# SouthPoleTelescope/CosmoMC

Hardware: AMD Instinct MI355X
Metric: fast-param likelihood evals/sec/node (plik_lite_TTTEEE ℓmax=2508); R-1 vs wall-clock (higher is better)
Workload: dtype f64; 1 GPU; plik_lite_TTTEEE + Planck2018 lensing fast-parameter Metropolis step (BASELINE configs[2] minus lowl): GetProposalFast + native plik_lite (613 bins, l<=2508, full binning + quadratic form) + CMBlikes lensing (9 bins, linear correction) + calPlanck prior + accept; walkers_per_gpu=1024, stream_groups=1, global_walkers=1024, nbins=613, lmax=2508, parallelism=walkers sharded over 1 rank(s), no per-step collective

## Files before the change

cosmomc_amd/_native.py:

```python
from __future__ import annotations

import ctypes as C
import os
import re
import subprocess

PKG = os.path.dirname(os.path.abspath(__file__))
ROOT = os.path.dirname(PKG)
LIB_PATH = os.environ.get("COSMOMC_AMD_LIB") or os.path.join(PKG, "lib", "libcosmomc_amd.so")
HEADER = os.path.join(ROOT, "include", "cosmomc_amd.h")

CMBL_LOGZERO = 1e30
N_FIELDS = 10

ERRORS = {0: "OK", -1: "bad argument", -2: "I/O error", -3: "format error", -4: "numerical error",
          -5: "HIP error", -6: "unsupported"}


class NativeError(RuntimeError):
    def __init__(self, code, msg):
        super().__init__(f"[{ERRORS.get(code, code)}] {msg}")
        self.code = code


# ... 75 lines not shown
        L.cmbl_clik_workspace_size.restype = sz
        L.cmbl_status.argtypes = [vp, C.POINTER(i), i]
        L.cmbs_walker_seed.argtypes = [i, i, i, C.POINTER(i), C.POINTER(i)]
        L.cmbs_create.argtypes = [C.POINTER(CmbsConfig), C.POINTER(vp), C.c_char_p, sz]
        L.cmbs_destroy.argtypes = [vp]
        L.cmbs_last_error.argtypes = [vp]
        L.cmbs_last_error.restype = C.c_char_p
        L.cmbs_set_covariance.argtypes = [vp, vp]
        L.cmbs_set_test_gaussian.argtypes = [vp, vp, vp]
        L.cmbs_add_likelihood.argtypes = [vp, vp, vp, vp, ll, ll]
        L.cmbs_set_start.argtypes = [vp, vp, vp]
        L.cmbs_step.argtypes = [vp, i, i, vp]
        L.cmbs_set_groups.argtypes = [vp, i]
        L.cmbs_set_binned_cache.argtypes = [vp, i]
        L.cmbs_history_host.argtypes = [vp, i, i, vp]
        L.cmbs_set_trial_theory.argtypes = [vp, i, vp, ll, ll]
        L.cmbs_step_drag.argtypes = [vp, i, d, THEORY_FN, vp, vp]
        L.cmbs_step_theory.argtypes = [vp, i, THEORY_FN, vp, vp]
        L.cmbs_refresh_theory.argtypes = [vp, THEORY_FN, vp, vp]
        L.cmbt_create.argtypes = [C.POINTER(CmbtConfig), C.POINTER(vp), C.c_char_p, sz]
        L.cmbt_destroy.argtypes = [vp]
        L.cmbt_last_error.argtypes = [vp]
        L.cmbt_last_error.restype = C.c_char_p
        L.cmbt_eval.argtypes = [vp, i, vp, ll, i, vp, ll, ll, vp, vp]
        L.cmbt_set_derived.argtypes = [vp, C.POINTER(CmbtDerivedConfig)]
        L.cmbt_derived_count.argtypes = [vp]
        L.cmbt_derived_eval.argtypes = [vp, i, vp, ll, i, vp, ll, vp, vp]
        L.cmbs_set_theory_calculator.argtypes = [vp, vp]
        L.cmbs_set_like_calculator.argtypes = [vp, i, vp]
        L.cmbg_create.argtypes = [vp, C.POINTER(CmbgConfig), C.POINTER(vp), C.c_char_p, sz]
        L.cmbg_destroy.argtypes = [vp]
        L.cmbg_last_error.argtypes = [vp]
        L.cmbg_last_error.restype = C.c_char_p
        L.cmbg_eval.argtypes = [vp, i, vp, ll, i, vp, vp, vp]
        L.cmbs_add_derived_likelihood.argtypes = [vp, vp]
        L.cmbs_collector_enable.argtypes = [vp, i]
        L.cmbs_collector_add.argtypes = [vp, vp, i, i, i, vp]
        L.cmbs_collector_state_host.argtypes = [vp, vp, vp, vp, vp]
        L.cmbs_collector_thin.argtypes = [vp, i, vp]
        L.cmbs_collector_moments.argtypes = [vp, vp, vp, vp]
        L.cmbs_collector_limits.argtypes = [vp, vp, i, d, vp, vp]
        L.cmbs_chain_moments.argtypes = [vp, i, i, vp, vp, vp]
        L.cmbs_enable_history.argtypes = [vp, i]
        L.cmbs_history_stats.argtypes = [vp, i, i, vp, vp, vp]
        L.cmbs_history_count.argtypes = [vp]
        L.cmbs_state.argtypes = [vp, C.POINTER(vp), C.POINTER(vp), C.POINTER(vp), C.POINTER(vp)]
        L.cmbs_get_state_host.argtypes = [vp, vp, vp, vp, vp]
        L.cmbs_state_bytes.argtypes = [vp]
        L.cmbs_state_bytes.restype = sz
        L.cmbs_save_state.argtypes = [vp, vp, sz]
        L.cmbs_load_state.argtypes = [vp, vp, sz]
        L.cmbs_history_restore.argtypes = [vp, i, i, vp, vp]
        L.cmbs_history_terms_host.argtypes = [vp, i, i, vp]
        L.cmbl_profile_enable.argtypes = [i]
        L.cmbl_profile_reset.argtypes = []
        L.cmbl_profile_read.argtypes = [C.c_char_p, C.POINTER(d), C.POINTER(ll)]
        _lib = L
    return _lib


def exported_symbols_from_header() -> list[str]:
    with open(HEADER) as f:
        txt = f.read()
    txt = re.sub(r"/\*.*?\*/", "", txt, flags=re.S)
    return sorted(set(re.findall(r"\b(cmb[ls]_[a-z_0-9]+)\s*\(", txt)))


def check(rc: int, handle=None, kind: str = "cmbl"):
    if rc != 0:
        msg = ""
        if handle is not None:
            fn = {"cmbl": lib().cmbl_last_error, "cmbs": lib().cmbs_last_error, "cmbt": lib().cmbt_last_error,
                  "cmbg": lib().cmbg_last_error}[kind]
            msg = (fn(handle) or b"").decode()
        raise NativeError(rc, msg)


def current_stream_ptr(device=None) -> int:
    import torch
    if device is None:
        try:
            return torch._C._cuda_getCurrentRawStream(torch._C._cuda_getDevice())
        except AttributeError:
            pass
    return torch.cuda.current_stream(device).cuda_stream


def require_gpu():
    import torch
    if not torch.cuda.is_available():
        raise RuntimeError("cosmomc_amd compute needs an MI355X (HIP) device; none visible")


def profile_enable(on: bool = True):
    lib().cmbl_profile_enable(int(on))


def profile_reset():
    lib().cmbl_profile_reset()


def profile_read(kernel: str):
    t, n = C.c_double(), C.c_longlong()
    lib().cmbl_profile_read(kernel.encode(), C.byref(t), C.byref(n))
    return t.value, n.value
```

cosmomc_amd/csrc/mhbody.h:

```cpp
#pragma once

template <bool ACCEPT, bool PROPOSE>
__device__ __forceinline__ void mh_body(const DevCfg &c, int fast_only, double *hist_row, double *hist_terms, int blk0,
                                        double *lds, int bx, const TailWait *tw = nullptr)
{
    if (c.lean.on) {
        mh_lean<ACCEPT, PROPOSE>(c, hist_row, hist_terms, blk0, lds, bx, tw);
        return;
    }
    const Rows &R = c.rows;
    const int lane = threadIdx.x % MB, grp = threadIdx.x / MB;
    const int wl64 = threadIdx.x & 63, wave = threadIdx.x >> 6, nwave = MH_THREADS / 64;
    const int wb = (blk0 + bx) * MB;
    const int w = wb + lane;
    const bool act = w < c.W;
    const size_t W = c.ld;
    const int nlk = (c.n_like + 1) & ~1;
    const int nd_st = c.stage_R ? R.ND : R.ND - R.RR;
    const int ni_st = c.stage_cyc ? R.NI : R.CYC;
    const int ntd = c.stage_cov ? c.tl.n_dbl : c.tl.covinv;
    double *sd = lds;
    double *lk = sd + (size_t)nd_st * MB;
    double *vc = lk + (size_t)nlk * MB;
    double *tq = vc + (size_t)c.max_blk * MB;
    double *dq = tq + (size_t)c.tq_rows * MB;
    double *td = dq + (size_t)c.def_cap * (QF_GROUPS + 1) * MB;
    int *si = reinterpret_cast<int *>(td + ((ntd + 31) & ~31));
    int *it = si + (size_t)ni_st * MB;
    int *ti = it + (size_t)(c.stage_cyc ? c.all_n : 0) * MB;
    int *oobw = ti + ((c.tl.n_int + 63) & ~63);
    double *zz = reinterpret_cast<double *>(oobw + MB);
    int *ndw = reinterpret_cast<int *>(zz + (size_t)c.np * MB);
    int *i0w = ndw + MB;
    if (threadIdx.x < MB) oobw[threadIdx.x] = 0;
    if (PROPOSE && c.rot_defer && bx == 0 && threadIdx.x == 0)
        c.rot_cnt[2 * (blk0 * MB / 64) + (c.rot_par ^ 1)] = 0;
    const bool skipR = !c.stage_R;
#define SROW(r) ((skipR && (r) >= R.R) ? (r) - R.RR : (r))

    STAMP(0);
    const int rEnd = R.R + R.RR;
    if (skipR) {
        dma_rows_f64(sd, 0, c.sd, 0, R.R, W, wb, wl64, wave, nwave);
        dma_rows_f64(sd, R.R, c.sd, rEnd, R.ND - rEnd, W, wb, wl64, wave, nwave);
    } else {
        dma_rows_f64(sd, 0, c.sd, 0, R.ND, W, wb, wl64, wave, nwave);
    }
    dma_rows_i32(si, c.si, ni_st, W, wb, wl64, wave, nwave);
    dma_words(td, c.tab_d, 2 * ntd, wl64, wave, nwave);
    dma_words(ti, c.tab_i, c.tl.n_int, wl64, wave, nwave);
    const bool pre_col = PROPOSE && fast_only && !c.stage_R && c.pre_blk >= 0;
    constexpr int NRQ = (MAXBLK + NV - 1) / NV;
    double rq[NRQ];
    int col = -1, ncol = 0;
    const bool rq_early = pre_col && c.pre_lp >= 0;
    if (rq_early && act) {
        ncol = c.pre_n;
        if (c.pre_lp % ncol != 0) col = c.pre_off + c.pre_lp;
#pragma unroll
        for (int u = 0; u < NRQ; u++) {
// ... 302 lines not shown
```

cosmomc_amd/csrc/mhlean.h:

```cpp
#pragma once

template <bool ACCEPT, bool PROPOSE>
__device__ __forceinline__ void mh_lean(const DevCfg &c, double *hist_row, double *hist_terms, int blk0, double *lds,
                                        int bx, const TailWait *tw)
{
    const Rows &R = c.rows;
    const LeanCfg &L = c.lean;
    const int lane = threadIdx.x % MB, grp = threadIdx.x / MB;
    const int wl64 = threadIdx.x & 63, wave = threadIdx.x >> 6, nwave = MH_THREADS / 64;
    const int wb = (blk0 + bx) * MB;
    const int w = wb + lane;
    const bool act = w < c.W;
    const size_t W = c.ld;
    const int np = c.np;
    const int nd_lo = R.R, nd_hi = R.ND - R.P;
    double *sd = lds;
    double *sp = sd + (size_t)nd_lo * MB;
    double *dq = sp + (size_t)nd_hi * MB;
    double *zz = dq + (size_t)MAXDEF * (QF_GROUPS + 1) * MB;
    int *si = reinterpret_cast<int *>(zz + (size_t)np * MB);
    int *oobw = si + 8 * MB;
    int *ndw = oobw + MB;
    int *i0w = ndw + MB;
    if (threadIdx.x < MB) oobw[threadIdx.x] = 0;
    if (PROPOSE && c.rot_defer && bx == 0 && threadIdx.x == 0)
        c.rot_cnt[2 * (blk0 * MB / 64) + (c.rot_par ^ 1)] = 0;

    STAMP(0);
    dma_rows_f64(sd, 0, c.sd, 0, nd_lo, W, wb, wl64, wave, nwave);
    dma_rows_f64(sd, nd_lo, c.sd, R.P, nd_hi, W, wb, wl64, wave, nwave);
    dma_rows_i32(si, c.si, 8, W, wb, wl64, wave, nwave);
    constexpr int PG = MAXP / NV;
    double lo[PG], hi[PG], mu[PG], sg[PG];
    const double *td = c.tab_d;
#pragma unroll
    for (int u = 0; u < PG; u++) {
        const int i = grp + u * NV;
        if (ACCEPT && i < np) {
            lo[u] = td[c.tl.pmin + i];
            hi[u] = td[c.tl.pmax + i];
            mu[u] = td[c.tl.pmean + i];
            sg[u] = td[c.tl.pstd + i];
        }
    }
    int pu[PG];
    if (ACCEPT && hist_row) {
#pragma unroll
        for (int u = 0; u < PG; u++) {
            const int i = grp + u * NV;
            if (i < c.n_used) pu[u] = c.tab_i[c.tl.params_used + i];
        }
    }
    if (tw) tail_wait(*tw, wb / 64);
    if (ACCEPT && c.n_def) {
        const int tile = wb / QF_TILE, col = wb % QF_TILE + lane;
        for (int d = 0; d < MAXDEF; d++) {
            if (d >= c.n_def) break;
            const double *tp = c.def_part[d] + (size_t)tile * c.def_items[d] * QF_TILE;
            double *row = dq + (size_t)d * (QF_GROUPS + 1) * MB;
            if (grp < QF_GROUPS) row[(size_t)grp * MB + lane] = qf_group_sum(tp, c.def_items[d], grp, col);
            if (grp == NV - 1) row[(size_t)QF_GROUPS * MB + lane] = (c.def_add[d] && act) ? c.def_add[d][w] : 0.0;
        }
    }
    double lk[MAXLIKE], ct[MAXLIKE];
    if (ACCEPT && grp == 0 && act) {
#pragma unroll
        for (int l = 0; l < MAXLIKE; l++)
            if (l < c.n_like) {
                lk[l] = c.like_terms[(size_t)l * W + w];
                if (hist_terms) ct[l] = c.cur_terms[(size_t)l * W + w];
            }
    }
    STAMP(1);
    asm volatile("s_waitcnt vmcnt(0)" ::: "memory");
    __syncthreads();
    const double *trial_l = sp + (size_t)np * MB + lane;
    if (ACCEPT && act) {
        int oob = 0;
#pragma unroll
        for (int u = 0; u < PG; u++) {
            const int i = grp + u * NV;
            if (i < np) {
                const double qv = trial_l[(size_t)i * MB];
                if (qv > hi[u] || qv < lo[u]) oob = 1;
                double z2 = 0.0;
                if (c.has_priors && sg[u] != 0.0) {
                    const double z = (qv - mu[u]) / sg[u];
                    z2 = z * z;
                }
                zz[(size_t)i * MB + lane] = z2;
            }
        }
        if (oob) atomicOr(&oobw[lane], 1);
    }
    if (ACCEPT) __syncthreads();
    STAMP(2);

    if (grp == 0 && act) {
        Rng r;
        r.u = Col<double>{sd + (size_t)R.U * MB + lane, MB};
        r.c = sd[(size_t)R.C * MB + lane];
        r.gset = sd[(size_t)R.G * MB + lane];
        r.i97 = si[(size_t)R.I97 * MB + lane];
        r.j97 = si[(size_t)R.J97 * MB + lane];
        r.iset = si[(size_t)R.ISET * MB + lane];
        r.nd = 0;
        const int i97_0 = r.i97;
        double *P = sp + lane;
        double *T = sp + (size_t)np * MB + lane;
        double cur = sp[(size_t)(2 * np) * MB + lane];
        double mult = sp[(size_t)(2 * np + 1) * MB + lane];
        int nacc = si[(size_t)R.NACC * MB + lane];
        bool moved = false;
        if (ACCEPT) {
            for (int d = 0; d < MAXDEF; d++) {
                if (d >= c.n_def) break;
                const double *row = dq + (size_t)d * (QF_GROUPS + 1) * MB;
                double v = qf_tree(row + lane, MB);
                if (c.def_add[d]) v = v + row[(size_t)QF_GROUPS * MB + lane];
                const int l = c.def_like[d];
#pragma unroll
                for (int q = 0; q < MAXLIKE; q++)
                    if (q == l) lk[q] = v;
                const_cast<double *>(c.like_terms)[(size_t)l * W + w] = v;
            }
            double like;
            if (oobw[lane]) like = LOGZERO;
            else {
                double main = 0.0;
                bool zero = false;
#pragma unroll
                for (int l = 0; l < MAXLIKE; l++)
                    if (l < c.n_like) {
                        if (lk[l] == LOGZERO) zero = true;
                        main += lk[l];
                    }
                if (zero) like = LOGZERO;
                else {
                    like = main / c.temperature;
                    if (c.has_priors) {
                        double pri = 0.0;
                        for (int i = 0; i < np; i++) pri += zz[(size_t)i * MB + lane];
                        like = like + (pri / 2.0) / c.temperature;
                    }
                }
            }
            bool acc = false;
            if (like != LOGZERO) {
                acc = cur > like;
                if (!acc) acc = (double)randexp1(r) > like - cur;
            }
            moved = acc;
            if (acc) {
                if (mult > 0) nacc += 1;
                mult = 1.0;
                for (int i = 0; i < np; i++) P[(size_t)i * MB] = T[(size_t)i * MB];
                cur = like;
#pragma unroll
                for (int l = 0; l < MAXLIKE; l++)
                    if (l < c.n_like) {
                        ct[l] = lk[l];
                        c.cur_terms[(size_t)l * W + w] = ct[l];
                    }
            } else {
                mult += 1.0;
            }
            c.si[(size_t)R.ACCF * W + w] = acc ? 1 : 0;
            c.si[(size_t)R.NACC * W + w] = nacc;
            c.sd[(size_t)R.L * W + w] = cur;
            c.sd[(size_t)R.M * W + w] = mult;
            if (hist_row) hist_row[(size_t)c.n_used * c.W + w] = cur;
            if (hist_terms) {
#pragma unroll
                for (int l = 0; l < MAXLIKE; l++)
                    if (l < c.n_like) hist_terms[(size_t)l * c.W + w] = ct[l];
            }
        }
        STAMP(3);
        if (PROPOSE) {
            if (!moved)
                for (int i = 0; i < np; i++) T[(size_t)i * MB] = P[(size_t)i * MB];
            (void)ranmar(r);
            const double r1 = (ranmar(r) - 0.5) >= 0.0 ? 1.0 : -1.0;
            double rf;
            if (ranmar(r) < 0.33) {
                rf = (double)randexp1(r);
            } else {
                rf = 0.0;
                const double g = gaussian1(r);
                rf += g * g;
                rf = sqrt(rf / 1);
            }
            const double scale = rf * c.propose_scale;
            const double v0 = r1 * scale;
#pragma unroll
            for (int j = 0; j < LEAN_MAXC; j++)
                if (j < L.nc) {
                    double s = 0.0;
                    s += L.map[j] * v0;
                    T[(size_t)L.chg[j] * MB] += s;
                }
            if (c.pub_on)
#pragma unroll
                for (int k = 0; k < 2; k++) {
                    const int pc = c.pub_pcal[k];
                    const double v = pc >= 0 ? T[(size_t)pc * MB] : 1.0;
                    __hip_atomic_store(c.calbuf + (size_t)k * W + w, v, __ATOMIC_RELAXED, __HIP_MEMORY_SCOPE_AGENT);
                    __hip_atomic_store(c.calbuf_next + (size_t)k * W + w,
                                       __longlong_as_double((long long)TP_PIPE_UNSET), __ATOMIC_RELAXED,
                                       __HIP_MEMORY_SCOPE_AGENT);
                }
            STAMP(4);
#pragma unroll
            for (int l = 0; l < MAXLIKE; l++)
#pragma unroll
                for (int q = 0; q < LEAN_MAXQ; q++)
                    if (l < c.n_like && q < L.nn[l])
                        c.like_nuis[l][(size_t)w * L.nn[l] + q] = T[(size_t)L.nuis[l][q] * MB];
            c.sd[(size_t)L.r_row * W + w] = r1;
            c.si[(size_t)(R.CYCLP + 2) * W + w] = 1;
            c.si[(size_t)L.cyc_row * W + w] = 1;
            c.si[(size_t)L.blklp_row * W + w] = 1;
            c.si[(size_t)R.PROT * W + w] = 0;
        }
        c.sd[(size_t)R.C * W + w] = r.c;
        c.sd[(size_t)R.G * W + w] = r.gset;
        c.si[(size_t)R.I97 * W + w] = r.i97;
        c.si[(size_t)R.J97 * W + w] = r.j97;
        c.si[(size_t)R.ISET * W + w] = r.iset;
        ndw[lane] = r.nd < 97 ? r.nd : 97;
        i0w[lane] = i97_0;
    }
    __syncthreads();
    STAMP(12);
    if (!act) return;
    {
        const int nd = ndw[lane], i0 = i0w[lane];
        for (int t = grp; t < nd; t += NV) {
            int p = i0 - 1 - t;
            if (p < 0) p += 97;
            c.sd[(size_t)(R.U + p) * W + w] = sd[(size_t)(R.U + p) * MB + lane];
        }
    }
    for (int i = grp; i < np; i += NV) {
        if (ACCEPT) c.sd[(size_t)(R.P + i) * W + w] = sp[(size_t)i * MB + lane];
        if (PROPOSE) c.sd[(size_t)(R.T + i) * W + w] = sp[(size_t)(np + i) * MB + lane];
    }
    if (ACCEPT && hist_row) {
#pragma unroll
        for (int u = 0; u < PG; u++) {
            const int i = grp + u * NV;
            if (i < c.n_used) hist_row[(size_t)i * c.W + w] = sp[(size_t)pu[u] * MB + lane];
        }
    }
    STAMP(5);
#ifdef CMAMD_STAMPS
    asm volatile("s_waitcnt vmcnt(0)" ::: "memory");
    STAMP(6);
#endif
}
```

cosmomc_amd/csrc/mhrng.h:

```cpp
#pragma once

template <class T> struct Col {
    T *p;
    int s;
    __device__ T &operator[](int i) const { return p[(size_t)i * s]; }
};


struct Rng {
    Col<double> u;
    double c;
    int i97, j97, iset;
    double gset;
    int nd = 0;
};

__device__ __forceinline__ double ranmar(Rng &r)
{
    double uni = r.u[r.i97 - 1] - r.u[r.j97 - 1];
    if (uni < 0.0) uni += 1.0;
    r.u[r.i97 - 1] = uni;
    if (--r.i97 == 0) r.i97 = 97;
    if (--r.j97 == 0) r.j97 = 97;
    r.nd++;
    const double cd = 7654321.0 / 16777216.0, cm = 16777213.0 / 16777216.0;
    r.c -= cd;
    if (r.c < 0.0) r.c += cm;
    uni -= r.c;
    if (uni < 0.0) uni += 1.0;
    return uni;
}

__device__ __forceinline__ double gaussian1(Rng &r)
{
    if (r.iset == 0) {
        double v1, v2, rr;
        do {
            v1 = 2.0 * ranmar(r) - 1.0;
            v2 = 2.0 * ranmar(r) - 1.0;
            rr = v1 * v1 + v2 * v2;
        } while (rr >= 1.0);
        const double fac = sqrt(-2.0 * log(rr) / rr);
        r.gset = v1 * fac;
        r.iset = 1;
        return v2 * fac;
    }
    r.iset = 0;
    return r.gset;
}

__device__ __forceinline__ float randexp1(Rng &r)
{
    const float alog2 = 0.6931471805599453f, a = 5.7133631526454228f, b = 3.4142135623730950f;
    const float c = -1.6734053240284925f, p = 0.9802581434685472f, aa = 5.6005707569738080f;
    const float bb = 3.3468106480569850f, hh = 0.0026106723602095f, dd = 0.0857864376269050f;
    float u = (float)ranmar(r);
    while (u <= 0.0f) u = (float)ranmar(r);
    float g = c;
    u = u + u;
    while (u < 1.0f) {
        g = g + alog2;
        u = u + u;
    }
    u = u - 1.0f;
    if (u <= p) return g + aa / (bb - u);
    for (;;) {
        u = (float)ranmar(r);
        const float y = a / (b - u);
        const float up = (float)ranmar(r);
        const float bu = b - u;
        if ((up * hh + dd) * (bu * bu) <= expf(-(y + c))) return g + y;
    }
}
```

cosmomc_amd/csrc/mhstep.h:

```cpp
#pragma once


static constexpr int UNI_WT = 4;

template <bool ACCEPT, bool PROPOSE>
__device__ __forceinline__ void mh_step_body(DevCfg &c, int fast_only, double *hist_row, double *hist_terms,
                                             StepTail &t, const int2 *__restrict__ rows, TailWait &tw, int nmh)
{
    extern __shared__ __attribute__((aligned(16))) double lds[];
    const int2 rr = rows[blockIdx.x >> 3];
    const int lb = rr.y * 8 + (blockIdx.x & 7);
    if (!ACCEPT && blockIdx.x == 0)
        for (int i = threadIdx.x; i < tw.ntiles; i += MH_THREADS) tw.cnt[i] = 0u;
#ifdef CMAMD_STAMPS
    const bool stamp = ACCEPT && threadIdx.x == 0 && blockIdx.x < 2048;
    const int slot = PROPOSE ? 0 : 1;
    if (stamp) {
        unsigned xcc;
        asm volatile("s_getreg_b32 %0, hwreg(HW_REG_XCC_ID)" : "=s"(xcc));
        g_uni_stamps[slot][blockIdx.x][0] = __builtin_amdgcn_s_memrealtime();
        g_uni_stamps[slot][blockIdx.x][2] = xcc & 15;
        g_uni_stamps[slot][blockIdx.x][4] = 0;
        g_uni_stamps[slot][blockIdx.x][5] = 0;
    }
    struct End {
        bool on;
        int role, slot;
        __device__ ~End() {
            if (on) {
                g_uni_stamps[slot][blockIdx.x][3] = __builtin_amdgcn_s_memrealtime();
                g_uni_stamps[slot][blockIdx.x][4] = role + 1;
            }
        }
    } end_{stamp, rr.x, slot};
#endif
    if (rr.x == TAIL_QF) {
        if (lb >= t.nq) return;
        int item_ix, tile;
        qf_place(lb, t.q.src.n_items, t.q.src.xcd_map, item_ix, tile);
        __builtin_amdgcn_s_setprio(2);
        qfs_body(lds, item_ix, tile, t.q);
        tail_arrive(tw, tile);
    } else if (rr.x == TAIL_GAUSS) {
        const int grows = (t.ng + 7) >> 3, q = (lb & 7) * grows + (lb >> 3);
        if (q >= t.ng) return;
        small_gauss_body<UNI_WT, true, true>(t.g, lds, q);
        tail_arrive(tw, q * UNI_WT / 64);
    } else if (rr.x == TAIL_PASS) {
        if (lb >= t.np) return;
        tp_vec_body<2, true, false>(t.tp, t.dl, t.ld_field, t.ld_walker, t.W, reinterpret_cast<char *>(lds), lb);
    } else if (lb < nmh) {
        __builtin_amdgcn_s_setprio(3);
        if (ACCEPT && t.fold_g) {
            small_gauss_body<MB, true, false>(t.g, lds, lb);
            asm volatile("s_waitcnt vmcnt(0)" ::: "memory");
            __syncthreads();
#ifdef CMAMD_STAMPS
            if (threadIdx.x == 0 && blockIdx.x < 2048)
                g_uni_stamps[PROPOSE ? 0 : 1][blockIdx.x][5] = __builtin_amdgcn_s_memrealtime();
#endif
        }
        mh_body<ACCEPT, PROPOSE>(c, fast_only, hist_row, hist_terms, 0, lds, lb, ACCEPT ? &tw : nullptr);
    }
}
```

cosmomc_amd/csrc/sampler.h:

```cpp
#pragma once

#include "common.h"
#include "steptail.h"
#include "theorypass.h"

namespace cmamd {

static constexpr int MAXLIKE = 8;
static constexpr int MAXGROUPS = 8;
static constexpr int MAXDEF = 2;

struct Rows {
    int U = 0;
    int C = 97;
    int G = 98;
    int R = 100;
    int RR;
    int P, T, L, M;
    int ND;
    int I97 = 0, J97 = 1, ISET = 2, FASTIX = 3, NACC = 4;
    int CYCLP = 5;
    int BLKLP = 8;
    int ACCF;
    int PROT;
// ... 26 lines not shown
    int has_priors, test_like, n_lin;
    int rot_defer;
    int *rot_list;
    int *rot_cnt;
    int rot_par;
    int rot_serial;
    Rows rows;
    TabLayout tl;
    const int *tab_i;
    const double *tab_d;
    double *sd;
    int *si;
    int stage_R;
    int pre_blk;
    int pre_lp;
    int pre_off, pre_n;
    int stage_cyc;
    int stage_cov;
    int *itmp_g;
    int tq_rows;
    int n_like;
    const double *like_terms;
    double *cur_terms;
    int like_nidx[MAXLIKE], like_nn[MAXLIKE];
    double *like_nuis[MAXLIKE];
    unsigned long long like_dep[MAXLIKE];
    int mask_on;
    int *like_flag;
    const double *like_out[MAXLIKE];
    int def_cap;
    int n_def;
    int def_like[MAXDEF], def_items[MAXDEF];
    const double *def_part[MAXDEF];
    const double *def_add[MAXDEF];
    int pub_on;
    int pub_pcal[2];
    double *calbuf;
    double *calbuf_next;
    int bin_on, bin_nused, bin_Np, bin_cal;
    const double *bin_S, *bin_X;
    double *bin_delta;
};

struct TailWait {
    unsigned int *cnt;
    unsigned int epoch;
    unsigned int epoch_g;
    int nq_items;
    int ng, gwt;
    int *status;
    int nosignal;
    int stamp_slot;
    int ntiles;
};

struct TheoryView {
    const double *dl = nullptr;
    long long ld_field = 0, ld_walker = 0;
    bool operator==(const TheoryView &o) const {
        return dl == o.dl && ld_field == o.ld_field && ld_walker == o.ld_walker;
    }
};

struct LikeSlot {
    cmbl_t *like;
    std::vector<int> nidx;
    TheoryView th;
};

}

struct cmbg;

struct cmbs {
    cmamd::DevCfg dc{};
    int W = 0, np = 0, n_used = 0;
    std::vector<int> params_used;
    std::string last_error;
    cmamd::DevBuf rot;
    std::vector<int> rot_par;
    std::vector<int> rot_lp;
    bool rot_fast_any = false;
    int rot_fast_n = 0;
    int stage_R_force = -1;
    cmamd::DevBuf tab_i, tab_d, sd, si, like_terms, cur_terms, ws, hist, hist_terms, mom, itmp_g;
    cmamd::DevBuf nuis_bufs[cmamd::MAXLIKE];
    std::vector<int> h_tab_i;
    std::vector<double> h_tab_d;
    std::vector<cmamd::LikeSlot> likes;
    std::vector<cmbg *> dlikes;
    bool drv_cur = false;
    int n_rows() const { return (int)(likes.size() + dlikes.size()); }
    std::vector<int> indices, proposer_for_index, blk_start, blk_n, blk_nchanged, used_params_changed_all;
    std::vector<int> blk_changed_off, blk_map_off, blk_R_off, changed;
    int all_n = 0, slow_n = 0, fast_n = 0, nblocks = 0, R_total = 0, map_total = 0;
    size_t mh_lds = 0;
    int hist_cap = 0, hist_count = 0;
    bool started = false;
    int n_groups = 1;
    std::vector<int> grp0{0};
    hipStream_t streams[cmamd::MAXGROUPS] = {};
    hipEvent_t events[cmamd::MAXGROUPS + 1] = {};
    cmamd::DevBuf ws_g[cmamd::MAXGROUPS];
    cmamd::DevBuf drag_dd, drag_di, like_terms2;
    cmamd::DevBuf like_ws2[cmamd::MAXLIKE];
    bool no_drag_pair = false;
    bool drag_hbm = false;
    cmamd::DevBuf nuis_bufs2[cmamd::MAXLIKE];
    cmamd::TheoryView end_theory[cmamd::MAXLIKE];
    long long num_drag = 0;
    cmbt *calc = nullptr;
    cmamd::DevBuf calc_fail;
    cmbt *like_calc[cmamd::MAXLIKE] = {};
    cmamd::DevBuf calc_fail2;
    bool theory_moved = false, theory_stale = false;
    struct Collector {
        cmamd::DevBuf samp, state, flag, wcount, steps;
        int cap = 0;
        bool enabled = false;
    } coll;
    cmamd::DevBuf like_flag, like_cnt;
    cmamd::DevBuf like_outc[cmamd::MAXLIKE], like_nuisc[cmamd::MAXLIKE], like_dlc[cmamd::MAXLIKE];
    std::vector<int> sparse_likes;
    bool mask_on = false;
    std::vector<int> defer_likes;
    cmamd::DevBuf like_ws[cmamd::MAXLIKE];
    int pending_def = 0;
    std::unique_ptr<cmamd::TheoryPass> tpass;
    int tp_like[2] = {-1, -1};
    cmamd::WinStage tp_stage[2];
    bool no_corun = false;
    cmamd::DevBuf pipe_cal;
    unsigned pipe_epoch = 0;
    int pipe_ready = 0;
    int pipe_mode = 3;
    cmamd::DevBuf tail_S[2][2];
    cmamd::DevBuf tail_rowcal;
    int tail_ready = 0;
    int tail_qf = -1, tail_g = -1;
    cmamd::DevBuf tail_cnt;
    size_t tail_cnt_bytes = 0;
    unsigned tail_epoch = 0;
    unsigned tail_epoch_g = 0;
    cmamd::StepTailPlan uni_plan[3];
    size_t uni_lds = 0;
    int tail_nosignal = 0;
    bool binned_cache = false;
    int *pipe_status_host = nullptr;
    int *pipe_status_dev = nullptr;
    hipEvent_t pipe_ev = nullptr;
    bool pipe_ev_pending = false;
    cmamd::DevBuf bin_S;
    size_t bin_lds = 0;
    int tp_why = 0;
    bool lean_off = false;
    ~cmbs() {
        if (pipe_status_host) (void)hipHostFree(pipe_status_host);
        if (pipe_ev) (void)hipEventDestroy(pipe_ev);
        for (auto &st : streams)
            if (st) (void)hipStreamDestroy(st);
        for (auto &e : events)
            if (e) (void)hipEventDestroy(e);
    }
};

namespace cmamd {
void sampler_set_groups(cmbs *s, int n_groups);
void sampler_check_pipe(cmbs *s, bool wait = false);
void rot_schedule_unknown(cmbs *s);
void sampler_chain_moments(cmbs *s, int first, int last, const double *gmean, double *out, hipStream_t stream);
void sampler_history_host(cmbs *s, int first, int count, double *out);
void sampler_set_trial_theory(cmbs *s, int like_index, double *dl_end, long long ld_field, long long ld_walker);
void sampler_step_drag(cmbs *s, int n_steps, double dragging_steps, cmbs_theory_fn fn, void *user, hipStream_t stream);
void sampler_step_theory(cmbs *s, int n_steps, cmbs_theory_fn fn, void *user, hipStream_t stream);
void sampler_refresh_theory(cmbs *s, cmbs_theory_fn fn, void *user, hipStream_t stream);
void sampler_set_theory_calculator(cmbs *s, cmbt *calc);
void sampler_set_like_calculator(cmbs *s, int like_index, cmbt *calc);
void sampler_add_derived_likelihood(cmbs *s, cmbg *g);
void sampler_collector_enable(cmbs *s, int samp_capacity);
void sampler_collector_add(cmbs *s, const int *steps, int nsteps, int min_update, int check_burn, hipStream_t st);
void sampler_collector_state_host(cmbs *s, int *start, int *count, int *burn, int *thin);
void sampler_collector_thin(cmbs *s, int limit, hipStream_t st);
void sampler_collector_moments(cmbs *s, const double *gmean, double *out, hipStream_t stream);
void sampler_collector_limits(cmbs *s, const int *params, int ncheck, double limfrac, double *out, hipStream_t stream);
size_t sampler_collector_bytes(const cmbs *s);
void sampler_collector_save(cmbs *s, void *buf);
void sampler_collector_load(cmbs *s, const void *buf);
}
```

cosmomc_amd/csrc/sampler.hip:

```cpp
#include <algorithm>
#include <cmath>
#include <cstring>

#include <cstdlib>

#include "plikbin.h"
#include "qfs_body.h"
#include "quadform.h"
#include "sampler.h"
#include "smallgauss.h"
#include "theorycalc.h"
#ifdef CMAMD_STAMPS
namespace cmamd {
__device__ unsigned long long g_uni_stamps[2][2048][6];
}
#endif
#include "theorypass_body.h"

namespace cmamd {

static constexpr double LOGZERO = CMBL_LOGZERO;
static constexpr int MAXP = 64;
static constexpr int MAXBLK = 32;
static constexpr int NB = 64;
// ... 58 lines not shown
        return;
    }
    const int w = b - nmh_pad;
    for (int i = pb.nused + (int)threadIdx.x; i < pb.Np; i += MH_THREADS)
        c.bin_delta[(size_t)w * pb.Np + i] = 0.0;
    double acc[3][2] = {};
#pragma unroll
    for (int f = 0; f < 3; f++) {
        if (f > 0) __syncthreads();
        if (!plik_bin_products(pb, lds, w, f)) continue;
        const double *P = lds - pb.fr.lo[f];
#pragma unroll
        for (int k = 0; k < 2; k++) {
            const int i = pb.fr.b0[f] + (int)threadIdx.x + k * MH_THREADS;
            if (i < pb.fr.b1[f]) {
                const BinInfo bi = pb.bins[i];
                for (int l = bi.lmin; l <= bi.lmax; l++) acc[f][k] += P[l];
            }
        }
    }
    if (threadIdx.x == 0) {
        double cl;
        for (long it = 0;; it++) {
            cl = __hip_atomic_load(c.calbuf + w, __ATOMIC_RELAXED, __HIP_MEMORY_SCOPE_AGENT);
            if ((unsigned long long)__double_as_longlong(cl) != TP_PIPE_UNSET) break;
            if (it == (1l << 20)) {
                pipe_giveup(status);
                break;
            }
            __builtin_amdgcn_s_sleep(24);
        }
        cal_s = cl;
    }
    __syncthreads();
    const double cl = cal_s, c2 = cl * cl;
    const bool rot = (unsigned long long)__double_as_longlong(cl) == TP_PIPE_ROT;
    double *out = (rot ? const_cast<double *>(c.bin_S) : c.bin_delta) + (size_t)w * pb.Np;
#pragma unroll
    for (int f = 0; f < 3; f++)
#pragma unroll
        for (int k = 0; k < 2; k++) {
            const int i = pb.fr.b0[f] + (int)threadIdx.x + k * MH_THREADS;
            if (pb.fr.hi[f] >= pb.fr.lo[f] && i < pb.fr.b1[f]) out[i] = rot ? acc[f][k] : pb.X[i] - acc[f][k] / c2;
        }
}

#include "mhstep.h"

template <bool ACCEPT, bool PROPOSE>
__global__ __launch_bounds__(MH_THREADS, 3) void mh_step_kernel(DevCfg c, int fast_only, double *hist_row,
                                                                double *hist_terms, StepTail t,
                                                                const int2 *__restrict__ rows, TailWait tw, int nmh)
{
    mh_step_body<ACCEPT, PROPOSE>(c, fast_only, hist_row, hist_terms, t, rows, tw, nmh);
}

template <bool ACCEPT, bool PROPOSE>
__global__ __launch_bounds__(MH_THREADS, 3) void mh_tail_kernel(DevCfg c, int fast_only, double *hist_row,
                                                                double *hist_terms, StepTail t,
                                                                const int2 *__restrict__ rows, TailWait tw, int nmh)
{
    mh_step_body<ACCEPT, PROPOSE>(c, fast_only, hist_row, hist_terms, t, rows, tw, nmh);
}

#include "mhrot.h"
#include "mhdrag.h"

__global__ void start_kernel(DevCfg c)
{
    const int w = blockIdx.x * blockDim.x + threadIdx.x;
    if (w >= c.W) return;
    const size_t W = c.ld;
    const Tabs t = make_tabs(c, c.tab_i, c.tab_d);
    Col<double> q{c.sd + (size_t)c.rows.T * W + w, c.ld};
    Col<const double> lk{c.like_terms + w, c.ld};
    c.sd[(size_t)c.rows.L * W + w] = target_like(c, t, q, lk);
    for (int l = 0; l < c.n_like; l++) c.cur_terms[(size_t)l * W + w] = lk[l];
    for (int i = 0; i < c.np; i++) c.sd[(size_t)(c.rows.P + i) * W + w] = q[i];
    c.sd[(size_t)c.rows.M * W + w] = 0.0;
    c.si[(size_t)c.rows.NACC * W + w] = 0;
}

__global__ void gather_nuis(const double *trial, int W, int ld, const int *nidx, int n_nuis, double *out)
{
    const int w = blockIdx.x * blockDim.x + threadIdx.x;
    if (w >= W) return;
    for (int k = 0; k < n_nuis; k++) out[(size_t)w * n_nuis + k] = trial[(size_t)nidx[k] * ld + w];
}

struct SparseSet {
    int like[MAXLIKE], nn[MAXLIKE];
    double *nuisc[MAXLIKE];
    int *map[MAXLIKE];
};

__global__ __launch_bounds__(1024) void like_compact_kernel(DevCfg c, SparseSet ss, int *__restrict__ cnt)
{
    __shared__ int wsum[16];
    const int b = blockIdx.x, l = ss.like[b], nn = ss.nn[b];
    int *flag = c.like_flag + (size_t)l * c.ld;
    const double *nuis = c.like_nuis[l];
    const int t = threadIdx.x, lane = t & 63, wave = t >> 6;
    const int chunk = (c.W + 1023) / 1024, w0 = t * chunk, w1 = min(c.W, w0 + chunk);
    int n = 0;
    for (int w = w0; w < w1; w++) n += flag[w] != 0;
    int v = n;
    for (int o = 1; o < 64; o <<= 1) {
        const int y = __shfl_up(v, o);
        if (lane >= o) v += y;
    }
    if (lane == 63) wsum[wave] = v;
    __syncthreads();
    int before = 0;
    for (int q = 0; q < wave; q++) before += wsum[q];
    int off = before + v - n;
// ... 866 lines not shown

static StepTail make_tail(cmbs *s, int rd, int wr) {
    StepTail t;
    const int W = s->W;
    t.W = W;
    if (rd >= 0) {
        const int qi = s->tp_like[s->tail_qf], gi = s->tp_like[s->tail_g];
        Like &Q = *s->likes[qi].like->like;
        Like &G = *s->likes[gi].like->like;
        if (!Q.qf_source(t.q.src, W, s->like_ws[qi].p)) fail(CMBL_ERR_ARG, "internal: step tail quadratic form");
        t.q.S = s->tail_S[rd][s->tail_qf].as<double>();
        t.q.nuis = s->dc.like_nuis[qi];
        t.q.ld_nuis = std::max(1, Q.n_nuis);
        t.q.cal_index = s->tp_stage[s->tail_qf].cal_index;
        t.q.W = W;
        t.q.Wp = QuadForm::wpad(W);
        t.nq = t.q.src.n_items * (QuadForm::wpad(W) / QF_TILE);
        if (!G.corun_small(t.g, W, s->dc.like_nuis[gi], G.n_nuis, s->like_terms.as<double>() + (size_t)gi * s->dc.ld,
                           s->like_ws[gi].p))
            fail(CMBL_ERR_ARG, "internal: step tail chi^2");
        t.g.partial = s->tail_S[rd][s->tail_g].as<double>();
        t.g.row_cal = s->tail_rowcal.as<unsigned char>();
        t.g.stage_cal = s->tp_stage[s->tail_g].cal_index;
        t.ng = (W + UNI_WT - 1) / UNI_WT;
        t.fold_g = (wr >= 0 && t.g.d.nX <= MH_THREADS / MB) ? 1 : 0;
        if (t.fold_g) t.ng = 0;
    }
    if (wr >= 0) {
        TPOut o[2];
        for (int k = 0; k < 2; k++) {
            const int i = s->tp_like[k];
            const WinStage &st = s->tp_stage[k];
            Like &L = *s->likes[i].like->like;
            o[k] = TPOut{st.kind, st.cal_index, st.kind == 1 ? QuadForm::wpad(W) : st.ld, 0,
                         s->tail_S[wr][k].as<double>(), st.X, s->dc.like_nuis[i], (long long)std::max(1, L.n_nuis)};
        }
        t.tp = s->tpass->dev_args(o, W);
        const TheoryView &P = s->likes[s->tp_like[0]].th;
        t.dl = P.dl;
        t.ld_field = P.ld_field;
        t.ld_walker = P.ld_walker;
        t.np = s->tpass->n_blocks();
    }
    return t;
}

static void launch_unified(cmbs *s, hipStream_t stream, bool propose, int rd, int wr, const HistRow &row,
                           int fast_only) {
    const bool accept = rd >= 0;
    StepTail t = make_tail(s, rd, wr);
    DevCfg dc = s->dc;
    dc.mask_on = 0;
    dc.lean = lean_cfg(s, fast_only, false);
    dc.pub_on = 0;
    dc.n_def = 0;
    s->pending_def = 0;
    if (accept) {
        dc.n_def = 1;
        dc.def_like[0] = s->tp_like[s->tail_qf];
        dc.def_items[0] = t.q.src.n_items;
        dc.def_part[0] = t.q.src.partial;
        dc.def_add[0] = nullptr;
    }
    const int ng_rows = t.ng;
    TailWait tw{};
    tw.cnt = s->tail_cnt.as<unsigned int>();
    tw.epoch = s->tail_epoch + (accept ? 1u : 0u);
    tw.epoch_g = s->tail_epoch_g + ((accept && !t.fold_g) ? 1u : 0u);
    tw.nq_items = t.q.src.n_items;
    tw.ng = accept ? (s->W + UNI_WT - 1) / UNI_WT : 0;
    tw.gwt = UNI_WT;
    tw.status = s->pipe_status_dev;
    tw.nosignal = s->tail_nosignal;
    tw.stamp_slot = propose ? 0 : 1;
    tw.ntiles = (int)(s->tail_cnt_bytes / 4);
    const int nmh = (s->W + MB - 1) / MB;
    const int v = accept ? (propose ? 1 : 2) : 0;
    StepTailPlan &pl = s->uni_plan[v];
    if (pl.key[0] != t.nq || pl.key[1] != ng_rows || pl.key[2] != t.np) {
        const std::vector<int2> rows = tail_rows(t.nq, ng_rows, t.np, nmh);
        pl.d_rows.alloc(rows.size() * sizeof(int2));
        pl.d_rows.upload(rows.data(), rows.size() * sizeof(int2));
        pl.nrows = (int)rows.size();
        pl.key[0] = t.nq;
        pl.key[1] = ng_rows;
        pl.key[2] = t.np;
    }
    const dim3 grid((unsigned)pl.nrows * 8), b(MH_THREADS);
    const int2 *rows = pl.d_rows.as<int2>();
    static const char *names[3] = {"mh_step_first", "mh_step_kernel", "mh_step_last"};
    static const char *cnames[3] = {"mh_step_first", "mh_tail_kernel", "mh_tail_last"};
    const bool cached = s->binned_cache && accept && wr < 0 && rd == 0;
    try {
        timed_launch(cached ? cnames[v] : names[v], stream, [&](hipEvent_t e0, hipEvent_t e1) {
            if (cached && v == 1)
                hipExtLaunchKernelGGL(mh_tail_kernel<true, true>, grid, b, s->uni_lds, stream, e0, e1, 0, dc,
                                      fast_only, row.p, row.t, t, rows, tw, nmh);
            else if (cached && v == 2)
                hipExtLaunchKernelGGL(mh_tail_kernel<true, false>, grid, b, s->uni_lds, stream, e0, e1, 0, dc,
                                      fast_only, row.p, row.t, t, rows, tw, nmh);
            else if (v == 0)
                hipExtLaunchKernelGGL(mh_step_kernel<false, true>, grid, b, s->uni_lds, stream, e0, e1, 0, dc,
                                      fast_only, row.p, row.t, t, rows, tw, nmh);
            else if (v == 1)
                hipExtLaunchKernelGGL(mh_step_kernel<true, true>, grid, b, s->uni_lds, stream, e0, e1, 0, dc, fast_only,
                                      row.p, row.t, t, rows, tw, nmh);
            else
                hipExtLaunchKernelGGL(mh_step_kernel<true, false>, grid, b, s->uni_lds, stream, e0, e1, 0, dc,
                                      fast_only, row.p, row.t, t, rows, tw, nmh);
        });
        HIP_CHECK(hipGetLastError());
    } catch (...) {
        s->tail_ready = 0;
        pipe_status_post_nothrow(s, stream);
        throw;
    }
    if (accept) s->tail_epoch++;
    if (accept && !t.fold_g) s->tail_epoch_g++;
}

void sampler_step(cmbs *s, int n_steps, int fast_only, hipStream_t stream) {
    if (!s->started) fail(CMBL_ERR_ARG, "cmbs_set_start must be called before cmbs_step");
    check_theory_fresh(s);
    if (fast_only && s->fast_n == 0) fail(CMBL_ERR_ARG, "no fast parameters");
    if (!fast_only && s->slow_n > 0 && s->n_rows() > 0)
        fail(CMBL_ERR_ARG, "slow proposals need the theory at the trial point: use cmbs_step_theory");
    check_derived_calc(s, "cmbs_step");
    if (n_steps <= 0) return;
// ... 76 lines not shown

}

#ifdef CMAMD_STAMPS
extern "C" int cmamd_debug_uni_stamps(unsigned long long *host) {
    return hipMemcpyFromSymbol(host, HIP_SYMBOL(cmamd::g_uni_stamps), sizeof(cmamd::g_uni_stamps)) == hipSuccess ? 0
                                                                                                               : -5;
}
extern "C" int cmamd_debug_stamps(unsigned long long *host) {
    return hipMemcpyFromSymbol(host, HIP_SYMBOL(cmamd::g_stamps), sizeof(cmamd::g_stamps)) == hipSuccess ? 0 : -5;
}
#endif

extern "C" int cmamd_debug_rot_serial(cmbs *s, int mode) {
    if (!s) return -1;
    s->dc.rot_serial = mode;
    return 0;
}
extern "C" int cmamd_debug_stage_R(cmbs *s, int on) {
    if (!s) return -1;
    s->stage_R_force = on;
    cmamd::set_mh_lds(s);
    return 0;
}
extern "C" int cmamd_debug_tp_items(const cmbs *s, int *out, int cap) {
    if (!s || !s->tpass) return -1;
    const int n = std::min(cap, s->tpass->n_items());
    for (int k = 0; k < n; k++) {
        const cmamd::TPItem &it = s->tpass->item(k);
        const int v[6] = {it.field, it.l0, it.l1, it.nst, it.ncol, it.nsb};
        for (int q = 0; q < 6; q++) out[6 * k + q] = v[q];
    }
    return s->tpass->n_items();
}
extern "C" int cmamd_debug_tail_rows(int nq, int ng, int np, int nm, int *out, int cap) {
    const std::vector<int2> rows = cmamd::tail_rows(nq, ng, np, nm);
    const int n = std::min(cap, (int)rows.size());
    for (int k = 0; k < n; k++) {
        out[2 * k] = rows[k].x;
        out[2 * k + 1] = rows[k].y;
    }
    return (int)rows.size();
}
extern "C" int cmamd_debug_pipeline(cmbs *s, int mode) {
    if (!s || (mode != 0 && mode != 3)) return -1;
    s->pipe_mode = mode;
    return 0;
}
extern "C" int cmamd_debug_lean(cmbs *s, int on) {
    if (!s) return CMBL_ERR_ARG;
    s->lean_off = !on;
    return 0;
}
extern "C" int cmamd_debug_corun(cmbs *s, int on) {
    if (!s) return -1;
    s->no_corun = !on;
    return 0;
}
extern "C" int cmamd_debug_tail_nosignal(cmbs *s, int on) {
    if (!s) return -1;
    s->tail_nosignal = on;
    return 0;
}
extern "C" int cmamd_debug_drag_pair(cmbs *s, int on) {
    if (!s) return -1;
    s->no_drag_pair = on == 0;
    return 0;
}
extern "C" int cmamd_debug_drag_hbm(cmbs *s, int on) {
    if (!s) return -1;
    s->drag_hbm = on != 0;
    return 0;
}
extern "C" int cmamd_debug_pipe_status(cmbs *s) {
    if (!s || !s->pipe_status_host) return -1;
    if (hipDeviceSynchronize() != hipSuccess) return -1;
    return *reinterpret_cast<volatile int *>(s->pipe_status_host);
}
extern "C" int cmamd_debug_tail(const cmbs *s) { return s ? s->tail_ready : 0; }
extern "C" int cmamd_debug_fused(const cmbs *s) { return !s ? 0 : s->tpass ? s->tpass->n_items() : -s->tp_why; }
```

Before: 32.47 million evals/s.

## Precompute RANMAR random tape before tail wait to overlap RNG with likelihood tail

Before waiting on the likelihood tail, the lean MH kernel now precomputes up to 32 RANMAR draws per walker into LDS using a closed-form skip-ahead of the generator state. It then speculatively evaluates the accept exponential and both proposal-draw variants (accepted-path and rejected-path) in separate thread groups. After the wait, the accept/propose step picks the matching precomputed variant and advances the RNG state by the number of draws consumed. The aim is to move serial RNG latency off the critical path after tail_wait, at the cost of extra LDS, redundant draw computation, and a fallback path when the tape is invalid or too short.

```diff
diff --git a/cosmomc_amd/_native.py b/cosmomc_amd/_native.py
--- a/cosmomc_amd/_native.py
+++ b/cosmomc_amd/_native.py
@@ -151,6 +151,9 @@
         L.cmbs_load_state.argtypes = [vp, vp, sz]
         L.cmbs_history_restore.argtypes = [vp, i, i, vp, vp]
         L.cmbs_history_terms_host.argtypes = [vp, i, i, vp]
+        L.cmamd_debug_rng_tape.argtypes = [vp, i]
+        L.cmamd_debug_rng_tape_counts.argtypes = [vp, vp]
+        L.cmamd_debug_rng_tape_host.argtypes = [vp, d, i, i, i, vp, vp, vp]
         L.cmbl_profile_enable.argtypes = [i]
         L.cmbl_profile_reset.argtypes = []
         L.cmbl_profile_read.argtypes = [C.c_char_p, C.POINTER(d), C.POINTER(ll)]
diff --git a/cosmomc_amd/csrc/mhbody.h b/cosmomc_amd/csrc/mhbody.h
--- a/cosmomc_amd/csrc/mhbody.h
+++ b/cosmomc_amd/csrc/mhbody.h
@@ -1,11 +1,11 @@
 #pragma once
 
-template <bool ACCEPT, bool PROPOSE>
+template <bool ACCEPT, bool PROPOSE, bool TAPE = false>
 __device__ __forceinline__ void mh_body(const DevCfg &c, int fast_only, double *hist_row, double *hist_terms, int blk0,
                                         double *lds, int bx, const TailWait *tw = nullptr)
 {
     if (c.lean.on) {
-        mh_lean<ACCEPT, PROPOSE>(c, hist_row, hist_terms, blk0, lds, bx, tw);
+        mh_lean<ACCEPT, PROPOSE, TAPE>(c, hist_row, hist_terms, blk0, lds, bx, tw);
         return;
     }
     const Rows &R = c.rows;
diff --git a/cosmomc_amd/csrc/mhlean.h b/cosmomc_amd/csrc/mhlean.h
--- a/cosmomc_amd/csrc/mhlean.h
+++ b/cosmomc_amd/csrc/mhlean.h
@@ -1,6 +1,22 @@
 #pragma once
 
-template <bool ACCEPT, bool PROPOSE>
+template <class G> __device__ __forceinline__ void lean_draws(G &r, double &r1, double &rf)
+{
+    (void)ranmar(r);
+    r1 = (ranmar(r) - 0.5) >= 0.0 ? 1.0 : -1.0;
+    if (ranmar(r) < 0.33) {
+        rf = (double)randexp1(r);
+    } else {
+        rf = 0.0;
+        const double g = gaussian1(r);
+        rf += g * g;
+        rf = sqrt(rf / 1);
+    }
+}
+
+static constexpr size_t LEAN_TAPE_BYTES = (size_t)(3 * RNG_NT + 2 * 3) * MB * 8 + (size_t)(2 * 3 + 3) * MB * 4;
+
+template <bool ACCEPT, bool PROPOSE, bool TAPE>
 __device__ __forceinline__ void mh_lean(const DevCfg &c, double *hist_row, double *hist_terms, int blk0, double *lds,
                                         int bx, const TailWait *tw)
 {
@@ -22,6 +38,15 @@
     int *oobw = si + 8 * MB;
     int *ndw = oobw + MB;
     int *i0w = ndw + MB;
+    const bool tape = TAPE && ACCEPT && tw && tw->rng_nt > 0;
+    double *tx = reinterpret_cast<double *>(i0w + MB);
+    double *tr = tx + (size_t)RNG_NT * MB;
+    double *tc = tr + (size_t)RNG_NT * MB;
+    double *vd = tc + (size_t)RNG_NT * MB;
+    int *vi = reinterpret_cast<int *>(vd + (size_t)2 * 3 * MB);
+    float *e0w = reinterpret_cast<float *>(vi + (size_t)2 * 3 * MB);
+    int *nEw = reinterpret_cast<int *>(e0w + MB);
+    int *tpw = nEw + MB;
     if (threadIdx.x < MB) oobw[threadIdx.x] = 0;
     if (PROPOSE && c.rot_defer && bx == 0 && threadIdx.x == 0)
         c.rot_cnt[2 * (blk0 * MB / 64) + (c.rot_par ^ 1)] = 0;
@@ -51,25 +76,31 @@
             if (i < c.n_used) pu[u] = c.tab_i[c.tl.params_used + i];
         }
     }
-    if (tw) tail_wait(*tw, wb / 64);
-    if (ACCEPT && c.n_def) {
-        const int tile = wb / QF_TILE, col = wb % QF_TILE + lane;
-        for (int d = 0; d < MAXDEF; d++) {
-            if (d >= c.n_def) break;
-            const double *tp = c.def_part[d] + (size_t)tile * c.def_items[d] * QF_TILE;
-            double *row = dq + (size_t)d * (QF_GROUPS + 1) * MB;
-            if (grp < QF_GROUPS) row[(size_t)grp * MB + lane] = qf_group_sum(tp, c.def_items[d], grp, col);
-            if (grp == NV - 1) row[(size_t)QF_GROUPS * MB + lane] = (c.def_add[d] && act) ? c.def_add[d][w] : 0.0;
-        }
-    }
     double lk[MAXLIKE], ct[MAXLIKE];
-    if (ACCEPT && grp == 0 && act) {
-#pragma unroll
-        for (int l = 0; l < MAXLIKE; l++)
-            if (l < c.n_like) {
-                lk[l] = c.like_terms[(size_t)l * W + w];
-                if (hist_terms) ct[l] = c.cur_terms[(size_t)l * W + w];
-            }
+    auto term_loads = [&]() {
+        if (ACCEPT && c.n_def) {
+            const int tile = wb / QF_TILE, col = wb % QF_TILE + lane;
+            for (int d = 0; d < MAXDEF; d++) {
+                if (d >= c.n_def) break;
+                const double *tp = c.def_part[d] + (size_t)tile * c.def_items[d] * QF_TILE;
+                double *row = dq + (size_t)d * (QF_GROUPS + 1) * MB;
+                if (grp < QF_GROUPS) row[(size_t)grp * MB + lane] = qf_group_sum(tp, c.def_items[d], grp, col);
+                if (grp == NV - 1)
+                    row[(size_t)QF_GROUPS * MB + lane] = (c.def_add[d] && act) ? c.def_add[d][w] : 0.0;
+            }
+        }
+        if (ACCEPT && grp == 0 && act) {
+#pragma unroll
+            for (int l = 0; l < MAXLIKE; l++)
+                if (l < c.n_like) {
+                    lk[l] = c.like_terms[(size_t)l * W + w];
+                    if (hist_terms) ct[l] = c.cur_terms[(size_t)l * W + w];
+                }
+        }
+    };
+    if (!tape) {
+        if (tw) tail_wait(*tw, wb / 64);
+        term_loads();
     }
     STAMP(1);
     asm volatile("s_waitcnt vmcnt(0)" ::: "memory");
@@ -92,6 +123,50 @@
             }
         }
         if (oob) atomicOr(&oobw[lane], 1);
+    }
+    if (tape) {
+        {
+            const int i0 = si[(size_t)R.I97 * MB + lane], j0 = si[(size_t)R.J97 * MB + lane];
+            const double c0 = sd[(size_t)R.C * MB + lane];
+            double c1;
+            const bool ok = act && ranmar_tape_ok(i0, j0) && ranmar_carry(c0, 1, c1);
+            if (ok) {
+                const Col<const double> u{sd + (size_t)R.U * MB + lane, MB};
+                for (int n = grp; n < RNG_NT; n += NV) {
+                    double rn, cn, xn;
+                    ranmar_tape_draw(u, c0, i0, j0, n, rn, cn, xn);
+                    tr[(size_t)n * MB + lane] = rn;
+                    tc[(size_t)n * MB + lane] = cn;
+                    tx[(size_t)n * MB + lane] = xn;
+                }
+            }
+            __syncthreads();
+            static_assert(NV > 8, "the variants' thread groups");
+            const int var = grp == 4 ? 1 : grp == 8 ? 0 : -1;
+            if (act && var >= 0 && (var == 1 || PROPOSE)) {
+                TapeRng t{Col<const double>{tx + lane, MB}, min(tw->rng_nt, RNG_NT), si[(size_t)R.ISET * MB + lane],
+                          sd[(size_t)R.G * MB + lane]};
+                if (ok) {
+                    if (var == 1) {
+                        e0w[lane] = randexp1(t);
+                        nEw[lane] = t.nd;
+                    }
+                    if (PROPOSE) {
+                        double r1, rf;
+                        lean_draws(t, r1, rf);
+                        const double scale = rf * c.propose_scale;
+                        vd[(size_t)(var * 3 + 0) * MB + lane] = r1;
+                        vd[(size_t)(var * 3 + 1) * MB + lane] = r1 * scale;
+                        vd[(size_t)(var * 3 + 2) * MB + lane] = t.gset;
+                        vi[(size_t)(var * 3 + 0) * MB + lane] = t.iset;
+                        vi[(size_t)(var * 3 + 1) * MB + lane] = t.nd;
+                    }
+                }
+                vi[(size_t)(var * 3 + 2) * MB + lane] = (!ok || t.over) ? 1 : 0;
+            }
+        }
+        tail_wait(*tw, wb / 64);
+        term_loads();
     }
     if (ACCEPT) __syncthreads();
     STAMP(2);
@@ -112,6 +187,8 @@
         double mult = sp[(size_t)(2 * np + 1) * MB + lane];
         int nacc = si[(size_t)R.NACC * MB + lane];
         bool moved = false;
+        const bool use = tape && !vi[(size_t)(1 * 3 + 2) * MB + lane] && !(PROPOSE && vi[(size_t)2 * MB + lane]);
+        bool drew = false;
         if (ACCEPT) {
             for (int d = 0; d < MAXDEF; d++) {
                 if (d >= c.n_def) break;
@@ -148,7 +225,11 @@
             bool acc = false;
             if (like != LOGZERO) {
                 acc = cur > like;
-                if (!acc) acc = (double)randexp1(r) > like - cur;
+                if (!acc) {
+                    const float e0 = use ? e0w[lane] : randexp1(r);
+                    acc = (double)e0 > like - cur;
+                    drew = true;
+                }
             }
             moved = acc;
             if (acc) {
@@ -180,19 +261,20 @@
         if (PROPOSE) {
             if (!moved)
                 for (int i = 0; i < np; i++) T[(size_t)i * MB] = P[(size_t)i * MB];
-            (void)ranmar(r);
-            const double r1 = (ranmar(r) - 0.5) >= 0.0 ? 1.0 : -1.0;
-            double rf;
-            if (ranmar(r) < 0.33) {
-                rf = (double)randexp1(r);
+            double r1, v0;
+            if (use) {
+                const int var = drew ? 1 : 0;
+                r1 = vd[(size_t)(var * 3 + 0) * MB + lane];
+                v0 = vd[(size_t)(var * 3 + 1) * MB + lane];
+                r.gset = vd[(size_t)(var * 3 + 2) * MB + lane];
+                r.iset = vi[(size_t)(var * 3 + 0) * MB + lane];
+                r.nd = vi[(size_t)(var * 3 + 1) * MB + lane];
             } else {
-                rf = 0.0;
-                const double g = gaussian1(r);
-                rf += g * g;
-                rf = sqrt(rf / 1);
-            }
-            const double scale = rf * c.propose_scale;
-            const double v0 = r1 * scale;
+                double rf;
+                lean_draws(r, r1, rf);
+                const double scale = rf * c.propose_scale;
+                v0 = r1 * scale;
+            }
 #pragma unroll
             for (int j = 0; j < LEAN_MAXC; j++)
                 if (j < L.nc) {
@@ -223,6 +305,18 @@
             c.si[(size_t)L.blklp_row * W + w] = 1;
             c.si[(size_t)R.PROT * W + w] = 0;
         }
+        if (use) {
+            if (!PROPOSE) r.nd = drew ? nEw[lane] : 0;
+            if (r.nd) r.c = tc[(size_t)(r.nd - 1) * MB + lane];
+            r.i97 -= r.nd;
+            if (r.i97 <= 0) r.i97 += 97;
+            r.j97 -= r.nd;
+            if (r.j97 <= 0) r.j97 += 97;
+        }
+        if (tape) {
+            tpw[lane] = use ? 1 : 0;
+            if (tw->rng_cnt) tw->rng_cnt[(size_t)(use ? 0 : 1) * W + w] += 1;
+        }
         c.sd[(size_t)R.C * W + w] = r.c;
         c.sd[(size_t)R.G * W + w] = r.gset;
         c.si[(size_t)R.I97 * W + w] = r.i97;
@@ -236,10 +330,12 @@
     if (!act) return;
     {
         const int nd = ndw[lane], i0 = i0w[lane];
+        const bool from_tape = tape && tpw[lane];
         for (int t = grp; t < nd; t += NV) {
             int p = i0 - 1 - t;
             if (p < 0) p += 97;
-            c.sd[(size_t)(R.U + p) * W + w] = sd[(size_t)(R.U + p) * MB + lane];
+            const double *row = from_tape ? tr + (size_t)t * MB : sd + (size_t)(R.U + p) * MB;
+            c.sd[(size_t)(R.U + p) * W + w] = row[lane];
         }
     }
     for (int i = grp; i < np; i += NV) {
diff --git a/cosmomc_amd/csrc/mhrng.h b/cosmomc_amd/csrc/mhrng.h
--- a/cosmomc_amd/csrc/mhrng.h
+++ b/cosmomc_amd/csrc/mhrng.h
@@ -31,7 +31,61 @@
     return uni;
 }
 
-__device__ __forceinline__ double gaussian1(Rng &r)
+static constexpr int RNG_NT = 32;
+
+__host__ __device__ inline bool ranmar_carry(double c0, int k, double &ck)
+{
+    const long long CD = 7654321, CM = 16777213;
+    const double C = c0 * 16777216.0;
+    if (!(C >= 0.0 && C < (double)CM) || C != (double)(long long)C) return false;
+    long long v = ((long long)C - (long long)k * CD) % CM;
+    if (v < 0) v += CM;
+    ck = (double)v / 16777216.0;
+    return true;
+}
+
+__host__ __device__ inline bool ranmar_tape_ok(int i97, int j97)
+{
+    return i97 >= 1 && i97 <= 97 && j97 >= 1 && j97 <= 97 && (j97 - i97 + 97) % 97 == 33;
+}
+
+template <class U>
+__host__ __device__ inline bool ranmar_tape_draw(const U &u, double c0, int i97, int j97, int n, double &rn,
+                                                 double &cn, double &xn)
+{
+    int i = i97 - n, j = j97 - n;
+    if (i <= 0) i += 97;
+    if (j <= 0) j += 97;
+    double uni = u[i - 1] - u[j - 1];
+    if (uni < 0.0) uni += 1.0;
+    rn = uni;
+    if (!ranmar_carry(c0, n + 1, cn)) return false;
+    uni -= cn;
+    if (uni < 0.0) uni += 1.0;
+    xn = uni;
+    return true;
+}
+
+struct TapeRng {
+    Col<const double> x;
+    int nt;
+    int iset;
+    double gset;
+    int nd = 0;
+    bool over = false;
+};
+
+__device__ __forceinline__ double ranmar(TapeRng &r)
+{
+    const int n = r.nd++;
+    if (n >= r.nt) {
+        r.over = true;
+        return 0.5;
+    }
+    return r.x[n];
+}
+
+template <class G> __device__ __forceinline__ double gaussian1(G &r)
 {
     if (r.iset == 0) {
         double v1, v2, rr;
@@ -49,7 +103,7 @@
     return r.gset;
 }
 
-__device__ __forceinline__ float randexp1(Rng &r)
+template <class G> __device__ __forceinline__ float randexp1(G &r)
 {
     const float alog2 = 0.6931471805599453f, a = 5.7133631526454228f, b = 3.4142135623730950f;
     const float c = -1.6734053240284925f, p = 0.9802581434685472f, aa = 5.6005707569738080f;
diff --git a/cosmomc_amd/csrc/mhstep.h b/cosmomc_amd/csrc/mhstep.h
--- a/cosmomc_amd/csrc/mhstep.h
+++ b/cosmomc_amd/csrc/mhstep.h
@@ -3,7 +3,7 @@
 
 static constexpr int UNI_WT = 4;
 
-template <bool ACCEPT, bool PROPOSE>
+template <bool ACCEPT, bool PROPOSE, bool TAPE>
 __device__ __forceinline__ void mh_step_body(DevCfg &c, int fast_only, double *hist_row, double *hist_terms,
                                              StepTail &t, const int2 *__restrict__ rows, TailWait &tw, int nmh)
 {
@@ -60,6 +60,6 @@
                 g_uni_stamps[PROPOSE ? 0 : 1][blockIdx.x][5] = __builtin_amdgcn_s_memrealtime();
 #endif
         }
-        mh_body<ACCEPT, PROPOSE>(c, fast_only, hist_row, hist_terms, 0, lds, lb, ACCEPT ? &tw : nullptr);
+        mh_body<ACCEPT, PROPOSE, TAPE>(c, fast_only, hist_row, hist_terms, 0, lds, lb, ACCEPT ? &tw : nullptr);
     }
 }
diff --git a/cosmomc_amd/csrc/sampler.h b/cosmomc_amd/csrc/sampler.h
--- a/cosmomc_amd/csrc/sampler.h
+++ b/cosmomc_amd/csrc/sampler.h
@@ -102,6 +102,8 @@
     int nosignal;
     int stamp_slot;
     int ntiles;
+    int rng_nt;
+    int *rng_cnt;
 };
 
 struct TheoryView {
@@ -204,6 +206,8 @@
     size_t bin_lds = 0;
     int tp_why = 0;
     bool lean_off = false;
+    int rng_nt = 32;
+    cmamd::DevBuf rng_cnt;
     ~cmbs() {
         if (pipe_status_host) (void)hipHostFree(pipe_status_host);
         if (pipe_ev) (void)hipEventDestroy(pipe_ev);
diff --git a/cosmomc_amd/csrc/sampler.hip b/cosmomc_amd/csrc/sampler.hip
--- a/cosmomc_amd/csrc/sampler.hip
+++ b/cosmomc_amd/csrc/sampler.hip
@@ -134,7 +134,7 @@
                                                                 double *hist_terms, StepTail t,
                                                                 const int2 *__restrict__ rows, TailWait tw, int nmh)
 {
-    mh_step_body<ACCEPT, PROPOSE>(c, fast_only, hist_row, hist_terms, t, rows, tw, nmh);
+    mh_step_body<ACCEPT, PROPOSE, !(ACCEPT && PROPOSE)>(c, fast_only, hist_row, hist_terms, t, rows, tw, nmh);
 }
 
 template <bool ACCEPT, bool PROPOSE>
@@ -142,7 +142,7 @@
                                                                 double *hist_terms, StepTail t,
                                                                 const int2 *__restrict__ rows, TailWait tw, int nmh)
 {
-    mh_step_body<ACCEPT, PROPOSE>(c, fast_only, hist_row, hist_terms, t, rows, tw, nmh);
+    mh_step_body<ACCEPT, PROPOSE, true>(c, fast_only, hist_row, hist_terms, t, rows, tw, nmh);
 }
 
 #include "mhrot.h"
@@ -1115,6 +1115,8 @@
     DevCfg dc = s->dc;
     dc.mask_on = 0;
     dc.lean = lean_cfg(s, fast_only, false);
+    const bool tape_kernel = accept && (!propose || (s->binned_cache && wr < 0 && rd == 0));
+    const int rng_nt = (tape_kernel && dc.lean.on && lean_lds_bytes(s) + LEAN_TAPE_BYTES <= s->uni_lds) ? s->rng_nt : 0;
     dc.pub_on = 0;
     dc.n_def = 0;
     s->pending_def = 0;
@@ -1137,6 +1139,8 @@
     tw.nosignal = s->tail_nosignal;
     tw.stamp_slot = propose ? 0 : 1;
     tw.ntiles = (int)(s->tail_cnt_bytes / 4);
+    tw.rng_nt = rng_nt;
+    tw.rng_cnt = s->rng_cnt.as<int>();
     const int nmh = (s->W + MB - 1) / MB;
     const int v = accept ? (propose ? 1 : 2) : 0;
     StepTailPlan &pl = s->uni_plan[v];
@@ -1319,6 +1323,33 @@
     s->lean_off = !on;
     return 0;
 }
+extern "C" int cmamd_debug_rng_tape(cmbs *s, int nt) {
+    if (!s || nt < 0 || nt > cmamd::RNG_NT) return CMBL_ERR_ARG;
+    if (hipDeviceSynchronize() != hipSuccess) return CMBL_ERR_HIP;
+    try {
+        s->rng_cnt.alloc((size_t)2 * s->dc.ld * sizeof(int));
+    } catch (...) {
+        return CMBL_ERR_HIP;
+    }
+    s->rng_nt = nt;
+    return 0;
+}
+extern "C" int cmamd_debug_rng_tape_counts(cmbs *s, int *out) {
+    if (!s || !out || !s->rng_cnt.p) return CMBL_ERR_ARG;
+    if (hipDeviceSynchronize() != hipSuccess) return CMBL_ERR_HIP;
+    for (int k = 0; k < 2; k++)
+        if (hipMemcpy(out + (size_t)k * s->W, s->rng_cnt.as<int>() + (size_t)k * s->dc.ld, (size_t)s->W * sizeof(int),
+                      hipMemcpyDeviceToHost) != hipSuccess)
+            return CMBL_ERR_HIP;
+    return 0;
+}
+extern "C" int cmamd_debug_rng_tape_host(const double *u, double c, int i97, int j97, int n, double *r, double *cc,
+                                         double *x) {
+    if (!u || !r || !cc || !x || n < 0 || n > 97 || !cmamd::ranmar_tape_ok(i97, j97)) return CMBL_ERR_ARG;
+    for (int k = 0; k < n; k++)
+        if (!cmamd::ranmar_tape_draw(u, c, i97, j97, k, r[k], cc[k], x[k])) return CMBL_ERR_ARG;
+    return 0;
+}
 extern "C" int cmamd_debug_corun(cmbs *s, int on) {
     if (!s) return -1;
     s->no_corun = !on;
```

New measurement: 32.13 million evals/s. -1.0%, worse.
